# 2thleZ/flash_attention_metal

Hardware: AMD Instinct MI355X
Metric: attn_fwd_tflops (seqlen=4096, head_dim=64, bf16, causal) (higher is better)
Workload: dtype bf16; 1 GPU; BASELINE.json configs[2]: seqlen=4096 head_dim=64 batch=4 heads=16 bf16 is_causal=true per GPU; batch_per_gpu=4, heads=16, seq_len=4096, head_dim=64, is_causal=True

## Files before the change

### flash_attention_metal_amd/csrc/fa_mfma16_kernel.hip

```cpp
#include <stdlib.h>

#include <algorithm>

#include "fa_mfma_common.h"

#ifndef FA16_DEFER_THR
#define FA16_DEFER_THR 8.0f
#endif
#ifndef FA16_LAK
#define FA16_LAK (D == 128 ? 3 : 2)
#endif
#ifndef FA16_LAV
#define FA16_LAV (D == 128 ? 3 : 2)
#endif
#ifndef FA16_PRIO
#define FA16_PRIO 1
#endif
#ifndef FA16_ONES
#define FA16_ONES 1
#endif
#ifndef FA16_LAZY
#define FA16_LAZY 1
#endif
#ifndef FA16_LAZY_THR
#define FA16_LAZY_THR 0x1p20f
#endif
#ifndef FA16_LAZY_POISON
#define FA16_LAZY_POISON 0x1p64f
#endif
#ifndef FA16_LOOK
#define FA16_LOOK 1
#endif
#ifndef FA16_COLD
#define FA16_COLD 3
#endif
#ifndef FA16_TAIL
#define FA16_TAIL 1
#endif
#ifndef FA16_HALVES
#define FA16_HALVES 0
#endif
#ifndef FA16_BN128
#define FA16_BN128 64
#endif
#ifndef FA16_OCC128
#define FA16_OCC128 2
#endif
#ifndef FA16_SUB8
#define FA16_SUB8 1
#endif
#ifndef FA16_OCC
#define FA16_OCC 4
#endif

namespace fa {

typedef float f32x4 __attribute__((ext_vector_type(4)));

template <typename Tag> struct MT16;
template <> struct MT16<BF16> {
  using elem = __bf16;
  using vec8 = bf16x8;
  __device__ static __forceinline__ f32x4 mfma(vec8 a, vec8 b, f32x4 c) { return __builtin_amdgcn_mfma_f32_16x16x32_bf16(a, b, c, 0, 0, 0); }
};
template <> struct MT16<F16> {
  using elem = _Float16;
  using vec8 = f16x8;
  __device__ static __forceinline__ f32x4 mfma(vec8 a, vec8 b, f32x4 c) { return __builtin_amdgcn_mfma_f32_16x16x32_f16(a, b, c, 0, 0, 0); }
};

__device__ __forceinline__ float xlane(float x, int mask) { return __shfl_xor(x, mask, 64); }

template <typename Tag, int D, int SUB>
constexpr size_t mfma16_lds_bytes() {
  constexpr bool lazy = std::is_same<Tag, BF16>::value && D == 64 && (FA16_ONES != 0) && (FA16_LAZY == 1);
  return 4 * SUB * (size_t)(D == 128 ? FA16_BN128 : BN) * D * 2 + (lazy ? 16 : 0);
}

template <typename Tag, int D, bool CAUSAL, int RW, bool PAD, int SUB>
__device__ __forceinline__ void fwd_mfma16_body(const Params &p) {
  using M = MT16<Tag>;
  using vec8 = typename M::vec8;
  using elem = typename M::elem;
  constexpr int BMR = RW * WM;
  constexpr int RB = D * 2;
  constexpr int CPR = D / 8;
  constexpr int KS = D / 32;
  constexpr int DT = D / 16;
  constexpr int BNK = (D == 128) ? FA16_BN128 : BN;
  constexpr int KT = BNK / 16;
  constexpr int NKP = KT / 2;
  constexpr int TILE = BNK * RB;
  static_assert(D == 64 || D == 128, "head dims of the 16x16x32 kernel");

  extern __shared__ __attribute__((aligned(16))) char smem_generic[];
  lds_char *smem = (lds_char *)smem_generic;
  lds_char *Kbuf = smem;
  lds_char *Vbuf = smem + 2 * SUB * TILE;

  const int wave = __builtin_amdgcn_readfirstlane((int)threadIdx.x >> 6);
  const int lane = threadIdx.x & 63;
  const int c = lane & 15;
  const int g = lane >> 4;

  int bh, qb;
  map_block<CAUSAL>(blockIdx.x, p, bh, qb);
  long long base, base_kv;
  head_bases(bh, p, base, base_kv);
  const int coff = p.Nk - p.N;
  const int q0 = qb * BMR;
  const int qw0 = q0 + wave * WM;

  const int GRB = PAD ? p.D * 2 : RB;
  auto gcol = [&](int chunk) -> unsigned { return (!PAD || chunk * 8 < p.D) ? (unsigned)chunk * 16 : 0x80000000u; };
  const unsigned head_bytes = (unsigned)p.N * GRB, kv_head_bytes = (unsigned)p.Nk * GRB;
  const __amdgpu_buffer_rsrc_t rq = __builtin_amdgcn_make_buffer_rsrc((void *)((const char *)p.q + base * 2), 0, head_bytes, 0x00020000);
  const __amdgpu_buffer_rsrc_t rk = __builtin_amdgcn_make_buffer_rsrc((void *)((const char *)p.k + base_kv * 2), 0, kv_head_bytes, 0x00020000);
  const __amdgpu_buffer_rsrc_t rv = __builtin_amdgcn_make_buffer_rsrc((void *)((const char *)p.v + base_kv * 2), 0, kv_head_bytes, 0x00020000);

  vec8 qf[2][KS];
#pragma unroll
  for (int qt = 0; qt < 2; ++qt)
#pragma unroll
    for (int ks = 0; ks < KS; ++ks) {
      const u32x4 t = __builtin_amdgcn_raw_buffer_load_b128(rq, (unsigned)(qw0 + 16 * qt + c) * GRB + gcol(4 * ks + g), 0, 0);
      qf[qt][ks] = __builtin_bit_cast(vec8, t);
    }

  const int kx = (D == 64) ? ((c >> 1) & 7) : c;
  const lds_char *kptr[KS];
#pragma unroll
  for (int ks = 0; ks < KS; ++ks) {
    kptr[ks] = Kbuf + c * RB + (((4 * ks + g) ^ kx) << 4);
    asm volatile("" : "+v"(kptr[ks]));
  }
  const int vq = c >> 2, vp = c & 3;
  const int vrow = 4 * g + vq;
  const int vx = (D == 64) ? (((vrow >> 1) & 3) << 1) : ((vrow & 7) << 1);
  const lds_char *vptr[DT];
#pragma unroll
  for (int dt = 0; dt < DT; ++dt) {
    vptr[dt] = Vbuf + vrow * RB + ((((2 * dt) ^ vx) + (vp >> 1)) << 4) + 8 * (vp & 1);
    asm volatile("" : "+v"(vptr[dt]));
  }

  const int kv_end = CAUSAL ? min(p.Nk, q0 + BMR + coff) : p.Nk;
  const int nT = (kv_end + BNK - 1) / BNK;

  constexpr int RPP = 1024 / RB;
  constexpr int NPW = (BNK / RPP) / RW;
  static_assert((RW * RPP) % 16 == 0, "the piece stride must keep the swizzle");
  unsigned dma_kvo, dma_vvo;
  {
    const int row = wave * RPP + lane / CPR, pc = lane % CPR;
    const int skx = (D == 64) ? ((row >> 1) & 7) : (row & 15);
    const int svx = (D == 64) ? (((row >> 1) & 3) << 1) : ((row & 7) << 1);
    dma_kvo = (unsigned)(row * GRB) + gcol(pc ^ skx);
    dma_vvo = (unsigned)(row * GRB) + gcol(pc ^ svx);
  }
  auto stage_dma = [&](int t, int buf) {
#pragma unroll
    for (int j = 0; j < NPW; ++j) {
      const unsigned soff = PAD ? (unsigned)(t * BNK + j * RW * RPP) * GRB : (unsigned)t * TILE + j * (RW * 1024);
      const unsigned lk = (unsigned)(__UINTPTR_TYPE__)Kbuf + buf * TILE + (wave + RW * j) * 1024;
      const unsigned lv = (unsigned)(__UINTPTR_TYPE__)Vbuf + buf * TILE + (wave + RW * j) * 1024;
      asm volatile("s_mov_b32 m0, %0\n\ts_nop 0\n\tbuffer_load_dwordx4 %1, %2, %3 offen lds" ::"s"(lk), "v"(dma_kvo), "s"(rk), "s"(soff) : "memory");
      asm volatile("s_mov_b32 m0, %0\n\ts_nop 0\n\tbuffer_load_dwordx4 %1, %2, %3 offen lds" ::"s"(lv), "v"(dma_vvo), "s"(rv), "s"(soff) : "memory");
    }
  };

  f32x4 oacc[DT][2];
#pragma unroll
  for (int dt = 0; dt < DT; ++dt)
#pragma unroll
    for (int qt = 0; qt < 2; ++qt)
#pragma unroll
      for (int i = 0; i < 4; ++i) oacc[dt][qt][i] = 0.0f;
  constexpr bool ONES = (FA16_ONES != 0);
  constexpr bool LAZY = ONES && std::is_same<Tag, BF16>::value && D == 64 && (FA16_LAZY != 0);
  constexpr bool LAZY_TEST = LAZY && (FA16_LAZY == 1);
  constexpr bool LOOK_PV = LAZY_TEST && (FA16_LOOK == 1), LOOK_FRONT = LAZY_TEST && (FA16_LOOK == 0);
  constexpr bool COLD3 = LAZY_TEST && (FA16_COLD == 3);
  constexpr bool TAIL_OUT = LAZY_TEST && (FA16_TAIL == 1);
  static_assert(4 * SUB * TILE + (LAZY_TEST ? 4 : 0) <= mfma16_lds_bytes<Tag, D, SUB>() && RW * WM * RB <= 4 * SUB * TILE,
                "the launcher's LDS size covers the K / V buffers, the flag word and the epilogue's O tiles");
  lds_char *poison_flag = smem + 4 * SUB * TILE;
  int slow = 0;
  constexpr float BIAS = !ONES ? 0.0f : std::is_same<Tag, F16>::value ? 3.0f : 7.0f;
  constexpr float FIRST_SUM_FLOOR = std::is_same<Tag, F16>::value ? 1.0f : 0x1p-64f;
  float l[2] = {0.0f, 0.0f};
  f32x4 lacc[2];
#pragma unroll
  for (int qt = 0; qt < 2; ++qt)
#pragma unroll
    for (int i = 0; i < 4; ++i) lacc[qt][i] = 0.0f;
  vec8 ones;
#pragma unroll
  for (int j = 0; j < 8; ++j) ones[j] = (elem)1.0f;
  if constexpr (ONES) asm volatile("" : "+v"(ones));
  const float c2 = p.scale * 1.4426950408889634f;
  f32x4 negm[2];
#pragma unroll
  for (int qt = 0; qt < 2; ++qt) {
#pragma unroll
    for (int i = 0; i < 4; ++i) negm[qt][i] = ONES ? -BIAS : INFINITY;
    asm volatile("" : "+v"(negm[qt]));
  }

  if constexpr (LAZY_TEST) {
    if (threadIdx.x == 0) lds_write_b32(poison_flag, 0u);
  }
  stage_dma(0, 0);
  if constexpr (SUB == 2) {
    if (1 < nT) stage_dma(1, 1);
  }
  asm volatile("s_waitcnt vmcnt(0)" ::: "memory");
#pragma unroll
  for (int qt = 0; qt < 2; ++qt)
#pragma unroll
    for (int ks = 0; ks < KS; ++ks) {
#pragma unroll
      for (int j = 0; j < 8; ++j) qf[qt][ks][j] = (elem)((float)qf[qt][ks][j] * c2);
      asm volatile("" : "+v"(qf[qt][ks]));
    }
  __syncthreads();

  const float sum_thr = __builtin_exp2f(FA16_DEFER_THR);
  auto apply_mask = [&](auto k0c, auto &s, const int kv0) __attribute__((always_inline)) {
    constexpr int K0 = decltype(k0c)::value;
    constexpr int NKT = sizeof(s) / sizeof(s[0]);
    int g4 = 4 * g;
    asm volatile("" : "+v"(g4));
#pragma unroll
    for (int qt = 0; qt < 2; ++qt) {
      int lim = p.Nk - 1 - kv0 - g4;
      if (CAUSAL) lim = min(lim, qw0 + 16 * qt + c + coff - kv0 - g4);
#pragma unroll
      for (int k2 = 0; k2 < NKT; ++k2)
#pragma unroll
        for (int i = 0; i < 4; ++i) s[k2][qt][i] = (16 * (K0 + k2) + i > lim) ? -INFINITY : s[k2][qt][i];
    }
  };
  auto needs_mask = [&](const int kv0) __attribute__((always_inline)) { return (CAUSAL && (kv0 + BNK - 1 > qw0 + coff)) || (kv0 + BNK > p.Nk); };
  auto score_group = [&](auto bufc, auto k0c, auto &s, const f32x4 c0, const f32x4 c1) __attribute__((always_inline)) {
    constexpr int buf = decltype(bufc)::value;
    constexpr int K0 = decltype(k0c)::value;
    constexpr int NKT = sizeof(s) / sizeof(s[0]);
    constexpr int NK = NKT * KS, LA = (FA16_LAK < NK) ? FA16_LAK : NK;
    vec8 kf[NK];
    auto kread = [&](int i) { kf[i] = __builtin_bit_cast(vec8, lds_read_b128(kptr[i % KS] + buf * TILE + (K0 + i / KS) * 16 * RB)); };
#pragma unroll
    for (int i = 0; i < LA; ++i) kread(i);
    __builtin_amdgcn_sched_barrier(0);
#pragma unroll
    for (int i = 0; i < NK; ++i) {
      const int k2 = i / KS, ks = i % KS;
      s[k2][0] = M::mfma(kf[i], qf[0][ks], ks == 0 ? c0 : s[k2][0]);
      s[k2][1] = M::mfma(kf[i], qf[1][ks], ks == 0 ? c1 : s[k2][1]);
      if (i + LA < NK) kread(i + LA);
      __builtin_amdgcn_sched_barrier(0);
    }
  };
  auto pack_group = [&](auto k0c, auto &s, vec8 (&pf)[NKP][2], unsigned &bits) __attribute__((always_inline)) {
    constexpr int K0 = decltype(k0c)::value;
    constexpr int NKT = sizeof(s) / sizeof(s[0]);
#pragma unroll
    for (int kp = 0; kp < NKT / 2; ++kp)
#pragma unroll
      for (int qt = 0; qt < 2; ++qt) {
#pragma unroll
        for (int j = 0; j < 8; ++j) pf[K0 / 2 + kp][qt][j] = (elem)s[2 * kp + (j >> 2)][qt][j & 3];
        if constexpr (ONES && !LAZY) {
          const u32x4 w = __builtin_bit_cast(u32x4, pf[K0 / 2 + kp][qt]);
          bits |= w[0] | w[1] | w[2] | w[3];
        }
      }
  };
  auto hot_group = [&](auto bufc, auto k0c, auto nktc, const int kv0, vec8 (&pf)[NKP][2], unsigned &bits, float (&ls)[2],
                       const bool leave, const int masked) __attribute__((always_inline)) -> bool {
    constexpr int NKT = decltype(nktc)::value;
    f32x4 s[NKT][2];
    score_group(bufc, k0c, s, negm[0], negm[1]);
    if constexpr (COLD3) {
      if (masked < 0) apply_mask(k0c, s, kv0);
    } else {
      if constexpr (LAZY_TEST && FA16_COLD != 2) {
        if (__builtin_expect(leave, 0)) return true;
      }
      if (needs_mask(kv0)) apply_mask(k0c, s, kv0);
    }
#if FA16_PRIO
    if constexpr (decltype(k0c)::value + NKT == KT) __builtin_amdgcn_s_setprio(0);
#endif
#pragma unroll
    for (int k2 = 0; k2 < NKT; ++k2)
#pragma unroll
      for (int i = 0; i < 4; ++i)
#pragma unroll
        for (int qt = 0; qt < 2; ++qt) {
          s[k2][qt][i] = __builtin_amdgcn_exp2f(s[k2][qt][i]);
          if constexpr (!ONES) ls[qt] = (decltype(k0c)::value == 0 && k2 == 0 && i == 0) ? s[k2][qt][i] : ls[qt] + s[k2][qt][i];
        }
    pack_group(k0c, s, pf, bits);
    return false;
  };
  auto max_group = [&](auto bufc, auto k0c, auto nktc, const int kv0, float (&mx)[2], const int masked) __attribute__((always_inline)) {
    constexpr int NKT = decltype(nktc)::value;
    f32x4 s[NKT][2], zero;
#pragma unroll
    for (int i = 0; i < 4; ++i) zero[i] = 0.0f;
    score_group(bufc, k0c, s, zero, zero);
    if (COLD3 ? masked < 0 : needs_mask(kv0)) apply_mask(k0c, s, kv0);
#pragma unroll
    for (int qt = 0; qt < 2; ++qt)
#pragma unroll
      for (int k2 = 0; k2 < NKT; ++k2)
#pragma unroll
        for (int i = 0; i < 4; ++i) mx[qt] = fmaxf(mx[qt], s[k2][qt][i]);
  };
  auto new_reference = [&](auto firstc, float (&mx)[2]) __attribute__((always_inline)) {
    constexpr bool FIRST = decltype(firstc)::value;
#pragma unroll
    for (int qt = 0; qt < 2; ++qt) {
      float v = mx[qt];
      v = fmaxf(v, xlane(v, 16));
      v = fmaxf(v, xlane(v, 32));
      const float m_old = -negm[qt][0];
      const float m_new = FIRST ? v + BIAS : fmaxf(m_old, v + BIAS);
#pragma unroll
      for (int i = 0; i < 4; ++i) negm[qt][i] = -m_new;
      asm volatile("" : "+v"(negm[qt]));
      if constexpr (FIRST) continue;
      const float alpha = __builtin_amdgcn_exp2f(m_old - m_new);
      if constexpr (ONES) {
#pragma unroll
        for (int i = 0; i < 4; ++i) lacc[qt][i] *= alpha;
      } else {
        l[qt] *= alpha;
      }
#pragma unroll
      for (int dt = 0; dt < DT; ++dt)
#pragma unroll
        for (int i = 0; i < 4; ++i) oacc[dt][qt][i] *= alpha;
    }
  };
  constexpr unsigned LAZY_THR_BITS = __builtin_bit_cast(unsigned, (float)FA16_LAZY_THR);
  constexpr unsigned LAZY_POISON_BITS = __builtin_bit_cast(unsigned, (float)FA16_LAZY_POISON);
  static_assert(LAZY_THR_BITS < LAZY_POISON_BITS && LAZY_POISON_BITS < 0x7f800000u, "2^-BIAS << THR < POISON < inf");
  auto lazy_look = [&]() __attribute__((always_inline)) -> unsigned long long {
    const unsigned b0 = __builtin_bit_cast(unsigned, lacc[0][0]), b1 = __builtin_bit_cast(unsigned, lacc[1][0]);
    return __builtin_amdgcn_ballot_w64(max(b0, b1) >= LAZY_THR_BITS);
  };
  auto lazy_repair = [&]() __attribute__((always_inline)) {
#pragma unroll
    for (int qt = 0; qt < 2; ++qt) {
      const unsigned a = __builtin_bit_cast(unsigned, lacc[qt][0]) & 0x7fffffffu;
      const bool bad = a >= LAZY_POISON_BITS;
      const bool big = !bad && a >= LAZY_THR_BITS;
      const int e = (int)(a >> 23) - 127;
      const float sc = big ? __builtin_bit_cast(float, (unsigned)(127 - e) << 23) : 1.0f;
      const float kf = big ? (float)e : 0.0f;
#pragma unroll
      for (int i = 0; i < 4; ++i) {
        lacc[qt][i] *= sc;
        negm[qt][i] -= kf;
      }
      asm volatile("" : "+v"(negm[qt]));
#pragma unroll
      for (int dt = 0; dt < DT; ++dt)
#pragma unroll
        for (int i = 0; i < 4; ++i) oacc[dt][qt][i] *= sc;
      if (bad) lds_write_b32(poison_flag, 1u);
    }
  };
  constexpr int G = (FA16_HALVES != 0) ? 2 : 1;
  using KTG = std::integral_constant<int, KT / G>;
  using K0A = std::integral_constant<int, 0>;
  using K0B = std::integral_constant<int, KT / 2>;

  auto tile = [&](auto bufc, auto firstc, const int t) {
    constexpr int buf = decltype(bufc)::value;
    constexpr bool FIRST = decltype(firstc)::value;
    const int kv0 = t * BNK;

    int always = 1;
    if constexpr (!CAUSAL) asm volatile("" : "+s"(always));
    const bool wave_active = CAUSAL ? (kv0 <= qw0 + WM - 1 + coff) : (always != 0);
    if (wave_active) {
      vec8 pf[NKP][2];
      float ls[2] = {0.0f, 0.0f};
      if constexpr (LOOK_FRONT && !FIRST) {
        if (__builtin_expect(lazy_look() != 0, 0)) lazy_repair();
      }
      int masked = 0;
      if constexpr (COLD3) {
        const int to_diagonal = CAUSAL ? (qw0 + coff) - (kv0 + BNK - 1) : 0, to_end = p.Nk - (kv0 + BNK);
        masked = to_diagonal | to_end;
        asm volatile("" : "+s"(masked));
      }
      unsigned long long look = 0;
      bool redo = (FIRST && !ONES) || (COLD3 && slow != 0);
      for (;;) {
        if (__builtin_expect(redo, 0)) {
          float mx[2] = {-INFINITY, -INFINITY};
          max_group(bufc, K0A{}, std::integral_constant<int, KT / 2>{}, kv0, mx, masked);
          max_group(bufc, K0B{}, std::integral_constant<int, KT / 2>{}, kv0, mx, masked);
          new_reference(firstc, mx);
        }
#if FA16_PRIO
        __builtin_amdgcn_s_setprio(1);
#endif
        unsigned bits = 0;
        if constexpr (LAZY_TEST) {
          if (hot_group(bufc, K0A{}, KTG{}, kv0, pf, bits, ls, !COLD3 && slow != 0 && !redo, masked)) {
            redo = true;
            continue;
          }
        } else {
          hot_group(bufc, K0A{}, KTG{}, kv0, pf, bits, ls, false, 0);
        }
        if constexpr (G == 2) hot_group(bufc, K0B{}, KTG{}, kv0, pf, bits, ls, false, 0);
        bool stale;
        if constexpr (LAZY) stale = false;
        else if constexpr (ONES) stale = __builtin_amdgcn_ballot_w64((bits & 0x40004000u) != 0) != 0;
        else stale = __builtin_amdgcn_ballot_w64(fmaxf(ls[0], ls[1]) > sum_thr) != 0;
        if (__builtin_expect(stale && !redo, 0)) {
          redo = true;
          continue;
        }
        if constexpr (!ONES) {
          l[0] += ls[0];
          l[1] += ls[1];
        }
#if FA16_PRIO
        __builtin_amdgcn_s_setprio(1);
#endif
        {
          constexpr int NV = NKP * DT, LA = FA16_LAV;
          s16x4 wlo[NV], whi[NV];
          auto vread = [&](int j) {
            const lds_char *vb = vptr[j % DT] + buf * TILE + (32 * (j / DT)) * RB;
            wlo[j] = lds_read_tr16(vb);
            whi[j] = lds_read_tr16(vb + 16 * RB);
          };
#pragma unroll
          for (int j = 0; j < LA; ++j) vread(j);
          __builtin_amdgcn_sched_barrier(0);
#pragma unroll
          for (int j = 0; j < NV; ++j) {
            const s16x8 v8 = __builtin_shufflevector(wlo[j], whi[j], 0, 1, 2, 3, 4, 5, 6, 7);
#pragma unroll
            for (int qt = 0; qt < 2; ++qt) oacc[j % DT][qt] = M::mfma(__builtin_bit_cast(vec8, v8), pf[j / DT][qt], oacc[j % DT][qt]);
            if (j + LA < NV) vread(j + LA);
            if constexpr (ONES) {
              if (j % DT == DT - 1) {
#pragma unroll
                for (int qt = 0; qt < 2; ++qt) lacc[qt] = M::mfma(ones, pf[j / DT][qt], lacc[qt]);
              }
            }
            if constexpr (LOOK_PV && !FIRST) {
              if (j == 0) {
                look = lazy_look();
                asm volatile("" : "+s"(look));
              }
            }
            __builtin_amdgcn_sched_barrier(0);
          }
        }
#if FA16_PRIO
        __builtin_amdgcn_s_setprio(0);
#endif
        if constexpr (LOOK_PV && !FIRST) {
          if (__builtin_expect(look != 0, 0)) lazy_repair();
        }
        if constexpr (FIRST && ONES) {
          if (__builtin_expect(!redo && __builtin_amdgcn_ballot_w64(fminf(lacc[0][0], lacc[1][0]) < FIRST_SUM_FLOOR) != 0, 0)) {
#pragma unroll
            for (int qt = 0; qt < 2; ++qt) {
#pragma unroll
              for (int i = 0; i < 4; ++i) lacc[qt][i] = 0.0f;
#pragma unroll
              for (int dt = 0; dt < DT; ++dt)
#pragma unroll
                for (int i = 0; i < 4; ++i) oacc[dt][qt][i] = 0.0f;
            }
            redo = true;
            continue;
          }
        }
        break;
      }
    }
  };
  auto tail_test = [&]() __attribute__((always_inline)) {
    const unsigned a0 = __builtin_bit_cast(unsigned, lacc[0][0]) & 0x7fffffffu, a1 = __builtin_bit_cast(unsigned, lacc[1][0]) & 0x7fffffffu;
    if (max(a0, a1) >= LAZY_POISON_BITS) lds_write_b32(poison_flag, 1u);
  };
  auto unit = [&](auto bufc, auto firstc, const int t0) {
    constexpr int buf = decltype(bufc)::value;
#pragma unroll
    for (int sub = 0; sub < SUB; ++sub)
      if (t0 + SUB + sub < nT) stage_dma(t0 + SUB + sub, (buf ^ 1) * SUB + sub);
    tile(std::integral_constant<int, buf * SUB>{}, firstc, t0);
    if constexpr (SUB == 2) {
      if (t0 + 1 < nT) tile(std::integral_constant<int, buf * SUB + 1>{}, std::false_type{}, t0 + 1);
    }
    if constexpr (TAIL_OUT) {
      if (t0 + SUB < nT) {
        asm volatile("s_waitcnt vmcnt(0)" ::: "memory");
        __syncthreads();
      }
    } else {
      if (t0 + SUB < nT) asm volatile("s_waitcnt vmcnt(0)" ::: "memory");
      if constexpr (LAZY_TEST) {
        if (t0 + SUB >= nT && slow == 0) tail_test();
      }
      __syncthreads();
    }
  };
  for (;;) {
    unit(std::integral_constant<int, 0>{}, std::true_type{}, 0);
    for (int t = SUB; t < nT; t += 2 * SUB) {
      unit(std::integral_constant<int, 1>{}, std::false_type{}, t);
      if (t + SUB < nT) unit(std::integral_constant<int, 0>{}, std::false_type{}, t + SUB);
    }
    if constexpr (TAIL_OUT) {
      if (slow == 0) tail_test();
      __syncthreads();
    }
    if constexpr (LAZY_TEST) {
      if (slow == 0) {
        const unsigned f = *reinterpret_cast<const volatile __attribute__((address_space(3))) unsigned *>(poison_flag);
        if (__builtin_expect(__builtin_amdgcn_readfirstlane((int)f) != 0, 0)) {
          slow = 1;
#pragma unroll
          for (int qt = 0; qt < 2; ++qt) {
#pragma unroll
            for (int i = 0; i < 4; ++i) {
              lacc[qt][i] = 0.0f;
              negm[qt][i] = -BIAS;
            }
            asm volatile("" : "+v"(negm[qt]));
#pragma unroll
            for (int dt = 0; dt < DT; ++dt)
#pragma unroll
              for (int i = 0; i < 4; ++i) oacc[dt][qt][i] = 0.0f;
          }
          stage_dma(0, 0);
          if constexpr (SUB == 2) {
            if (1 < nT) stage_dma(1, 1);
          }
          asm volatile("s_waitcnt vmcnt(0)" ::: "memory");
          __syncthreads();
          continue;
        }
      }
    }
    break;
  }

  int elane = lane;
  if constexpr (LAZY_TEST) asm volatile("" : "+v"(elane));
  const int ec = elane & 15, eg = elane >> 4;
  lds_char *Ot = smem + wave * (WM * RB);
#pragma unroll
  for (int qt = 0; qt < 2; ++qt) {
    float lt = ONES ? lacc[qt][0] : l[qt];
    if constexpr (!ONES) {
      lt += xlane(lt, 16);
      lt += xlane(lt, 32);
    }
    const float inv_l = __builtin_amdgcn_rcpf(lt);
    const int row = 16 * qt + ec, qrow = qw0 + row;
    if (p.lse != nullptr && eg == 0 && qrow < p.N)
      p.lse[(long long)bh * p.N + qrow] = (__builtin_amdgcn_logf(lt) - negm[qt][0]) * 0.6931471805599453f;
#pragma unroll
    for (int dt = 0; dt < DT; ++dt) {
      typedef elem elem4 __attribute__((ext_vector_type(4)));
      elem4 e;
#pragma unroll
      for (int i = 0; i < 4; ++i) e[i] = (elem)(oacc[dt][qt][i] * inv_l);
      const u32x2 w = __builtin_bit_cast(u32x2, e);
      const int ch = (2 * dt + (eg >> 1)) ^ (row & (CPR - 1));
      lds_write_b64(Ot + row * RB + (ch << 4) + 8 * (eg & 1), w);
    }
  }
  __syncthreads();
  {
    elem *Og = (elem *)p.o + base;
#pragma unroll
    for (int it = 0; it < WM * CPR / 64; ++it) {
      const int idx = it * 64 + elane;
      const int row = idx / CPR, ch = idx % CPR;
      const u32x4 vv = lds_read_b128(Ot + row * RB + ((ch ^ (row & (CPR - 1))) << 4));
      if (qw0 + row < p.N && (!PAD || ch * 8 < p.D)) *reinterpret_cast<u32x4 *>(Og + (long long)(qw0 + row) * (PAD ? p.D : D) + ch * 8) = vv;
    }
  }
}

template <typename Tag, int D, bool CAUSAL, int RW, bool PAD = false, int SUB = 1>
__global__ __launch_bounds__(64 * RW, (D == 64 ? FA16_OCC : FA16_OCC128)) void fwd_mfma16_kernel(Params p) {
  fwd_mfma16_body<Tag, D, CAUSAL, RW, PAD, SUB>(p);
}

bool mfma16_supported(int dtype, int D) { return (dtype == FA_DTYPE_F16 || dtype == FA_DTYPE_BF16) && D >= 8 && D <= 128 && D % 8 == 0; }

template <typename Tag, int D, bool CAUSAL, int RW, bool PAD = false, int SUB = 1>
static hipError_t launch16_one(const Params &p, hipStream_t s) {
  int head_group = causal_head_group(p, D, 2);
#ifdef FA16_FORCE_HEAD_GROUP
  head_group = FA16_FORCE_HEAD_GROUP;
#endif
  return launch_blocks(fwd_mfma16_kernel<Tag, D, CAUSAL, RW, PAD, SUB>, p, RW * WM, 64 * RW, mfma16_lds_bytes<Tag, D, SUB>(), head_group, s);
}

int mfma16_waves(int D, int BH, int N, int Nk, int is_causal) {
#ifdef FA16_FORCE_RW
  return FA16_FORCE_RW;
#endif
  if (D != 64 && D != 128) return 4;
  const long long b256 = (long long)BH * ((N + 255) / 256);
  if (D == 128) return (!is_causal && Nk >= 8192 && b256 >= 1024) ? 8 : 4;
  if (!is_causal) return (Nk >= 512 && b256 >= 512) ? 8 : 4;
  return (Nk >= 4096 && Nk < 6144 && b256 >= 1024 && b256 < 1280) ? 8 : 4;
}

hipError_t launch_mfma16(const Params &p, int dtype, hipStream_t s) {
  const bool w8 = mfma16_waves(p.D, p.B * p.H, p.N, p.Nk, p.is_causal) == 8 && (p.D == 64 || !p.is_causal);
  return with_tag(dtype, [&](auto tag) -> hipError_t {
    using Tag = decltype(tag);
    if (p.D != 64 && p.D != 128) {
      if (p.D < 64) return p.is_causal ? launch16_one<Tag, 64, true, 4, true>(p, s) : launch16_one<Tag, 64, false, 4, true>(p, s);
      return p.is_causal ? launch16_one<Tag, 128, true, 4, true>(p, s) : launch16_one<Tag, 128, false, 4, true>(p, s);
    }
    if (p.D == 64) {
      if (w8) return p.is_causal ? launch16_one<Tag, 64, true, 8, false, FA16_SUB8>(p, s) : launch16_one<Tag, 64, false, 8, false, FA16_SUB8>(p, s);
      return p.is_causal ? launch16_one<Tag, 64, true, 4>(p, s) : launch16_one<Tag, 64, false, 4>(p, s);
    }
    if (p.D == 128) {
      if (w8) return launch16_one<Tag, 128, false, 8>(p, s);
      return p.is_causal ? launch16_one<Tag, 128, true, 4>(p, s) : launch16_one<Tag, 128, false, 4>(p, s);
    }
    return hipErrorInvalidValue;
  });
}

}
```

Measured before the change: 1166 TFLOP/s.

## Issue first K/V DMA before Q loads and streamline the epilogue store

For D=64 with 8 waves, the first K/V tile DMA is now issued before the Q fragment loads, so the kernel prologue overlaps those global loads. For D=64 the epilogue drops the block-wide barrier in favor of a per-wave lgkmcnt wait, since each wave reads only its own O tile. It also writes O through buffer stores with a streaming/nontemporal cache hint instead of plain global stores. The changes risk a hazard if the per-wave LDS region assumption fails, and they touch only the prologue and epilogue.

After: 1176 TFLOP/s, median of 6. About the same (+0.9%).

```diff
diff --git a/flash_attention_metal_amd/csrc/fa_mfma16_kernel.hip b/flash_attention_metal_amd/csrc/fa_mfma16_kernel.hip
--- a/flash_attention_metal_amd/csrc/fa_mfma16_kernel.hip
+++ b/flash_attention_metal_amd/csrc/fa_mfma16_kernel.hip
@@ -51,6 +51,15 @@
 #endif
 #ifndef FA16_OCC
 #define FA16_OCC 4
+#endif
+#ifndef FA16_PRO
+#define FA16_PRO (D == 64 && RW == 8 ? 1 : 0)
+#endif
+#ifndef FA16_OST
+#define FA16_OST (D == 64 ? 1 : 0)
+#endif
+#ifndef FA16_EPB
+#define FA16_EPB (D == 64 ? 0 : 1)
 #endif
 
 namespace fa {
@@ -118,45 +127,22 @@
   const __amdgpu_buffer_rsrc_t rk = __builtin_amdgcn_make_buffer_rsrc((void *)((const char *)p.k + base_kv * 2), 0, kv_head_bytes, 0x00020000);
   const __amdgpu_buffer_rsrc_t rv = __builtin_amdgcn_make_buffer_rsrc((void *)((const char *)p.v + base_kv * 2), 0, kv_head_bytes, 0x00020000);
 
-  vec8 qf[2][KS];
-#pragma unroll
-  for (int qt = 0; qt < 2; ++qt)
-#pragma unroll
-    for (int ks = 0; ks < KS; ++ks) {
-      const u32x4 t = __builtin_amdgcn_raw_buffer_load_b128(rq, (unsigned)(qw0 + 16 * qt + c) * GRB + gcol(4 * ks + g), 0, 0);
-      qf[qt][ks] = __builtin_bit_cast(vec8, t);
-    }
-
-  const int kx = (D == 64) ? ((c >> 1) & 7) : c;
-  const lds_char *kptr[KS];
-#pragma unroll
-  for (int ks = 0; ks < KS; ++ks) {
-    kptr[ks] = Kbuf + c * RB + (((4 * ks + g) ^ kx) << 4);
-    asm volatile("" : "+v"(kptr[ks]));
-  }
-  const int vq = c >> 2, vp = c & 3;
-  const int vrow = 4 * g + vq;
-  const int vx = (D == 64) ? (((vrow >> 1) & 3) << 1) : ((vrow & 7) << 1);
-  const lds_char *vptr[DT];
-#pragma unroll
-  for (int dt = 0; dt < DT; ++dt) {
-    vptr[dt] = Vbuf + vrow * RB + ((((2 * dt) ^ vx) + (vp >> 1)) << 4) + 8 * (vp & 1);
-    asm volatile("" : "+v"(vptr[dt]));
-  }
-
-  const int kv_end = CAUSAL ? min(p.Nk, q0 + BMR + coff) : p.Nk;
-  const int nT = (kv_end + BNK - 1) / BNK;
+  auto count_tiles = [&]() __attribute__((always_inline)) {
+    const int kv_end = CAUSAL ? min(p.Nk, q0 + BMR + coff) : p.Nk;
+    return (kv_end + BNK - 1) / BNK;
+  };
 
   constexpr int RPP = 1024 / RB;
   constexpr int NPW = (BNK / RPP) / RW;
   static_assert((RW * RPP) % 16 == 0, "the piece stride must keep the swizzle");
   unsigned dma_kvo, dma_vvo;
-  {
-    const int row = wave * RPP + lane / CPR, pc = lane % CPR;
-    const int skx = (D == 64) ? ((row >> 1) & 7) : (row & 15);
-    const int svx = (D == 64) ? (((row >> 1) & 3) << 1) : ((row & 7) << 1);
-    dma_kvo = (unsigned)(row * GRB) + gcol(pc ^ skx);
-    dma_vvo = (unsigned)(row * GRB) + gcol(pc ^ svx);
+#define FA16_DMA_OFFSETS()                                                           \
+  {                                                                                  \
+    const int row = wave * RPP + lane / CPR, pc = lane % CPR;                        \
+    const int skx = (D == 64) ? ((row >> 1) & 7) : (row & 15);                       \
+    const int svx = (D == 64) ? (((row >> 1) & 3) << 1) : ((row & 7) << 1);          \
+    dma_kvo = (unsigned)(row * GRB) + gcol(pc ^ skx);                                \
+    dma_vvo = (unsigned)(row * GRB) + gcol(pc ^ svx);                                \
   }
   auto stage_dma = [&](int t, int buf) {
 #pragma unroll
@@ -168,6 +154,50 @@
       asm volatile("s_mov_b32 m0, %0\n\ts_nop 0\n\tbuffer_load_dwordx4 %1, %2, %3 offen lds" ::"s"(lv), "v"(dma_vvo), "s"(rv), "s"(soff) : "memory");
     }
   };
+  auto stage_first = [&](const int tiles) __attribute__((always_inline)) {
+    stage_dma(0, 0);
+    if constexpr (SUB == 2) {
+      if (1 < tiles) stage_dma(1, 1);
+    }
+  };
+
+  vec8 qf[2][KS];
+#define FA16_LOAD_Q()                                                                                                              \
+  _Pragma("unroll") for (int qt = 0; qt < 2; ++qt) _Pragma("unroll") for (int ks = 0; ks < KS; ++ks) {                             \
+    const u32x4 t = __builtin_amdgcn_raw_buffer_load_b128(rq, (unsigned)(qw0 + 16 * qt + c) * GRB + gcol(4 * ks + g), 0, 0);       \
+    qf[qt][ks] = __builtin_bit_cast(vec8, t);                                                                                      \
+  }
+  constexpr bool PRO = (FA16_PRO != 0);
+  if constexpr (PRO) {
+    FA16_DMA_OFFSETS();
+    stage_first(count_tiles());
+    FA16_LOAD_Q();
+    __builtin_amdgcn_sched_barrier(0);
+  } else {
+    FA16_LOAD_Q();
+  }
+#undef FA16_LOAD_Q
+
+  const int kx = (D == 64) ? ((c >> 1) & 7) : c;
+  const lds_char *kptr[KS];
+#pragma unroll
+  for (int ks = 0; ks < KS; ++ks) {
+    kptr[ks] = Kbuf + c * RB + (((4 * ks + g) ^ kx) << 4);
+    asm volatile("" : "+v"(kptr[ks]));
+  }
+  const int vq = c >> 2, vp = c & 3;
+  const int vrow = 4 * g + vq;
+  const int vx = (D == 64) ? (((vrow >> 1) & 3) << 1) : ((vrow & 7) << 1);
+  const lds_char *vptr[DT];
+#pragma unroll
+  for (int dt = 0; dt < DT; ++dt) {
+    vptr[dt] = Vbuf + vrow * RB + ((((2 * dt) ^ vx) + (vp >> 1)) << 4) + 8 * (vp & 1);
+    asm volatile("" : "+v"(vptr[dt]));
+  }
+
+  const int nT = count_tiles();
+  if constexpr (!PRO) FA16_DMA_OFFSETS();
+#undef FA16_DMA_OFFSETS
 
   f32x4 oacc[DT][2];
 #pragma unroll
@@ -210,11 +240,17 @@
   if constexpr (LAZY_TEST) {
     if (threadIdx.x == 0) lds_write_b32(poison_flag, 0u);
   }
-  stage_dma(0, 0);
-  if constexpr (SUB == 2) {
-    if (1 < nT) stage_dma(1, 1);
-  }
-  asm volatile("s_waitcnt vmcnt(0)" ::: "memory");
+  if constexpr (PRO) {
+    __builtin_amdgcn_sched_barrier(0);
+    asm volatile("s_waitcnt vmcnt(0)" ::: "memory");
+#pragma unroll
+    for (int qt = 0; qt < 2; ++qt)
+#pragma unroll
+      for (int ks = 0; ks < KS; ++ks) asm volatile("" : "+v"(qf[qt][ks]));
+  } else {
+    stage_first(nT);
+    asm volatile("s_waitcnt vmcnt(0)" ::: "memory");
+  }
 #pragma unroll
   for (int qt = 0; qt < 2; ++qt)
 #pragma unroll
@@ -563,6 +599,8 @@
   if constexpr (LAZY_TEST) asm volatile("" : "+v"(elane));
   const int ec = elane & 15, eg = elane >> 4;
   lds_char *Ot = smem + wave * (WM * RB);
+  [[maybe_unused]] int ost_never = 0;
+  if constexpr (FA16_OST == 3) asm volatile("" : "+s"(ost_never));
 #pragma unroll
   for (int qt = 0; qt < 2; ++qt) {
     float lt = ONES ? lacc[qt][0] : l[qt];
@@ -572,7 +610,7 @@
     }
     const float inv_l = __builtin_amdgcn_rcpf(lt);
     const int row = 16 * qt + ec, qrow = qw0 + row;
-    if (p.lse != nullptr && eg == 0 && qrow < p.N)
+    if (p.lse != nullptr && eg == 0 && qrow < p.N && (FA16_OST != 3 || ost_never != 0))
       p.lse[(long long)bh * p.N + qrow] = (__builtin_amdgcn_logf(lt) - negm[qt][0]) * 0.6931471805599453f;
 #pragma unroll
     for (int dt = 0; dt < DT; ++dt) {
@@ -585,8 +623,9 @@
       lds_write_b64(Ot + row * RB + (ch << 4) + 8 * (eg & 1), w);
     }
   }
-  __syncthreads();
-  {
+  if constexpr (FA16_EPB != 0) __syncthreads();
+  else asm volatile("s_waitcnt lgkmcnt(0)" ::: "memory");
+  if constexpr (FA16_OST == 0) {
     elem *Og = (elem *)p.o + base;
 #pragma unroll
     for (int it = 0; it < WM * CPR / 64; ++it) {
@@ -594,6 +633,18 @@
       const int row = idx / CPR, ch = idx % CPR;
       const u32x4 vv = lds_read_b128(Ot + row * RB + ((ch ^ (row & (CPR - 1))) << 4));
       if (qw0 + row < p.N && (!PAD || ch * 8 < p.D)) *reinterpret_cast<u32x4 *>(Og + (long long)(qw0 + row) * (PAD ? p.D : D) + ch * 8) = vv;
+    }
+  } else {
+    constexpr int aux = (FA16_OST == 2) ? 2 : 16;
+    const __amdgpu_buffer_rsrc_t ro = __builtin_amdgcn_make_buffer_rsrc((void *)((char *)p.o + base * 2), 0, head_bytes, 0x00020000);
+    if (FA16_OST != 3 || ost_never != 0) {
+#pragma unroll
+      for (int it = 0; it < WM * CPR / 64; ++it) {
+        const int idx = it * 64 + elane;
+        const int row = idx / CPR, ch = idx % CPR;
+        const u32x4 vv = lds_read_b128(Ot + row * RB + ((ch ^ (row & (CPR - 1))) << 4));
+        __builtin_amdgcn_raw_buffer_store_b128(vv, ro, (unsigned)(qw0 + row) * GRB + gcol(ch), 0, aux);
+      }
     }
   }
 }
```
